# iamwinter/UMPR

Measured on AMD Instinct MI355X. Metric: training samples/sec, higher is better.
Workload: dtype f32

## Files before the change

include/umpr_hip.h:

```cpp
#ifndef UMPR_HIP_H
#define UMPR_HIP_H
#include <stddef.h>
#include <stdint.h>

#ifdef __cplusplus
extern "C" {
#endif

const char* umpr_version(void);
const char* umpr_last_error(void);
int umpr_device_info(int dev, char* name, int name_len, int* compute_units, size_t* hbm_bytes);

int umpr_gemm_f32(const float* A, long lda, int transA, const float* B, long ldb, int transB, float* C, long ldc,
                  int M, int N, int K, const float* bias, int bias_mode, int act, int accumulate, float alpha,
                  float* ws, size_t ws_bytes, void* stream);

int umpr_set_gemm_bf16(int on);

int umpr_set_conv_inference(int on);

int umpr_set_conv_pool_follows(int on);

long umpr_debug_wino_fix_count(void);

int umpr_debug_conv3x3_plan(int pass, int N, int Cin, int Cout, int H, int W, int inference, size_t* ws_bytes, size_t* v_bytes);

int umpr_debug_wino_pool_fold(const float* y, const float* g_pooled, const float* w, const float* x, float* unpooled, float* dx,
                              float* dw, float* db, int N, int Cin, int Cout, int H, int W, int f4, int fold, float* ws,
                              size_t ws_bytes, void* stream);

size_t umpr_embed_gru_bidir_ws_bytes(int N, int L, int E);
int umpr_embed_gru_bidir_fwd(const int64_t* ids, const float* emb, int E,
                             const float* w_ih_f, const float* w_hh_f, const float* b_ih_f, const float* b_hh_f,
                             const float* w_ih_r, const float* w_hh_r, const float* b_ih_r, const float* b_hh_r,
                             const int32_t* lengths, const int32_t* order, const int32_t* dst_row, int N, int L,
                             float* out, float* saved, float* ws, size_t ws_bytes, void* stream);
int umpr_embed_gru_bidir_bwd(const int64_t* ids, const float* emb, int E,
                             const float* w_hh_f, const float* w_hh_r,
                             const int32_t* lengths, const int32_t* order, const int32_t* dst_row, int N, int L,
                             const float* dout, const float* out, const float* saved,
                             float* dw_ih_f, float* dw_hh_f, float* db_ih_f, float* db_hh_f,
                             float* dw_ih_r, float* dw_hh_r, float* db_ih_r, float* db_hh_r,
                             float* ws, size_t ws_bytes, void* stream);

int umpr_embed_gru_bidir_bwd_acc(const int64_t* ids, const float* emb, int E,
                                 const float* w_hh_f, const float* w_hh_r,
                                 const int32_t* lengths, const int32_t* order, const int32_t* dst_row, int N, int L,
                                 const float* dout, const float* out, const float* saved,
                                 float* dw_ih_f, float* dw_hh_f, float* db_ih_f, float* db_hh_f,
                                 float* dw_ih_r, float* dw_hh_r, float* db_ih_r, float* db_hh_r,
                                 int accumulate, float* ws, size_t ws_bytes, void* stream);

int umpr_embed_gru_bidir_bwd_dx(const int64_t* ids, const float* emb, int E,
                                const float* w_hh_f, const float* w_hh_r,
                                const int32_t* lengths, const int32_t* order, const int32_t* dst_row, int N, int L,
                                const float* dout, const float* out, const float* saved,
                                float* dw_ih_f, float* dw_hh_f, float* db_ih_f, float* db_hh_f,
                                float* dw_ih_r, float* dw_hh_r, float* db_ih_r, float* db_hh_r,
                                int accumulate, const float* w_ih_f, const float* w_ih_r, float* dx, int dx_accumulate,
                                float* ws, size_t ws_bytes, void* stream);

int umpr_embed_grad_chunk(void);
size_t umpr_embed_grad_ws_bytes(long T, int E);
int umpr_embed_grad(const int64_t* const* ids, const float* const* dx, const long* counts, int n_src, int E, long vocab,
                    const int32_t* sorted_pos, float* d_emb, void* ws, size_t ws_bytes, void* stream);

size_t umpr_embed_grad_rows_ws_bytes(long T, int E);
int umpr_embed_grad_rows(const int64_t* const* ids, const float* const* dx, const long* counts, int n_src, int E, long vocab,
                         const int32_t* sorted_pos, int64_t* row_id, float* row_grad, void* ws, size_t ws_bytes, void* stream);
int umpr_sparse_adam_rows(float* p, float* m, float* v, long vocab, int E, const int64_t* row_id, const float* row_grad, long T,
                          double lr, double beta1, double beta2, double eps, long step, double grad_scale,
                          const float* clip_state , void* stream);

size_t umpr_coattention_fwd_ws_bytes(int B, int SL);
int umpr_coattention_fwd(const float* Gu, const float* Gi, const float* M, int B, int SL, float* T, float* soft_u,
                         float* soft_i, float* atte_u, long ld_u, float* atte_i, long ld_i, float* colmax,
                         int32_t* argcol, float* rowmax, int32_t* argrow, float* ws, size_t ws_bytes, void* stream);
int umpr_coattention_fwd_bf16(const float* Gu, const float* Gi, const float* M, int B, int SL, float* T, float* soft_u,
                              float* soft_i, float* atte_u, long ld_u, float* atte_i, long ld_i, float* colmax,
                              int32_t* argcol, float* rowmax, int32_t* argrow, float* ws, size_t ws_bytes, void* stream);
int umpr_token_mask(const int64_t* ids, const int32_t* lengths, int N, int L, long pad_id, uint8_t* valid, void* stream);
int umpr_coattention_fwd_masked(const float* Gu, const float* Gi, const float* M, int B, int SL, float* T, float* soft_u,
                                float* soft_i, float* atte_u, long ld_u, float* atte_i, long ld_i, float* colmax,
                                int32_t* argcol, float* rowmax, int32_t* argrow, const uint8_t* valid_u,
                                const uint8_t* valid_i, int bf16_scores, float* ws, size_t ws_bytes, void* stream);
size_t umpr_coattention_bwd_ws_bytes(int B, int SL);
int umpr_coattention_bwd(const float* Gu, const float* Gi, const float* M, const float* T, const float* soft_u,
                         const float* soft_i, const float* colmax, const int32_t* argcol, const float* rowmax,
                         const int32_t* argrow, const float* d_atte_u, long ld_du, const float* d_atte_i, long ld_di,
                         const float* d_soft_u, const float* d_soft_i, int B, int SL, float* dGu, float* dGi,
                         float* dM, int accumulate , float* ws, size_t ws_bytes, void* stream);

int umpr_snet_fwd(const float* X, const float* Ms, const float* Ws, const float* word_soft, int wl, int B, int S,
                  int L, float* U, float* P, float* wsum, float* self_atte, float* senti, long ld_senti, void* stream);
int umpr_snet_fwd_masked(const float* X, const float* Ms, const float* Ws, const float* word_soft, int wl, int B, int S,
                         int L, float* U, float* P, float* wsum, float* self_atte, float* senti, long ld_senti,
                         const uint8_t* valid, void* stream);
size_t umpr_snet_bwd_ws_bytes(int B, int S, int L);
int umpr_snet_bwd(const float* X, const float* Ms, const float* Ws, const float* U, const float* P, const float* wsum,
                  const float* self_atte, const float* d_senti, long ld_ds, const float* d_self_atte ,
                  int B, int S, int L, int wl, float* dX, float* dMs, float* dWs, float* d_word_soft ,
                  float* ws, size_t ws_bytes, void* stream);

int umpr_review_merge_fwd(const float* repr_u, const float* repr_i, const float* W_u, const float* W_i, int B,
                          float* out, void* stream);
size_t umpr_review_merge_bwd_ws_bytes(int B);
int umpr_review_merge_bwd(const float* repr_u, const float* repr_i, const float* W_u, const float* W_i,
                          const float* out, const float* d_out, int B, float* d_repr_u, float* d_repr_i, float* dW_u,
                          float* dW_i, float* ws, size_t ws_bytes, void* stream);

size_t umpr_cnet_head_fwd_ws_bytes(int B, int S, int L, int KS);
int umpr_cnet_head_fwd(const float* X, const float* Wc, const float* bc, const float* Wl, const float* bl, float thr,
// ... 229 lines not shown
```

umpr_amd/_lib.py:

```python
from __future__ import annotations

import ctypes
import os
import threading

import torch

_HERE = os.path.dirname(os.path.abspath(__file__))
LIB_PATH = os.path.join(_HERE, "libumpr_hip.so")

_T = {"p": ctypes.c_void_p, "i": ctypes.c_int, "l": ctypes.c_long, "z": ctypes.c_size_t, "f": ctypes.c_float,
      "d": ctypes.c_double, "u": ctypes.c_uint64}

SIGNATURES = {
    "umpr_version": ("", "s"),
    "umpr_last_error": ("", "s"),
    "umpr_device_info": ("ipipp", "i"),
    "umpr_gemm_f32": ("pliplipliiipiiifpzp", "i"),
    "umpr_embed_gru_bidir_ws_bytes": ("iii", "z"),
    "umpr_embed_gru_bidir_fwd": ("ppipppppppppppiipppzp", "i"),
    "umpr_embed_gru_bidir_bwd": ("ppipppppiippppppppppppzp", "i"),
    "umpr_embed_gru_bidir_bwd_acc": ("ppipppppiipppppppppppipzp", "i"),
    "umpr_embed_gru_bidir_bwd_dx": ("ppipppppiipppppppppppipppipzp", "i"),
    "umpr_embed_grad_chunk": ("", "i"),
# ... 28 lines not shown
    "umpr_vgg16_fwd_ws_bytes": ("i", "z"),
    "umpr_vgg16_ws_bytes": ("i", "z"),
    "umpr_vgg16_fwd": ("ppiiiuppppzp", "i"),
    "umpr_vgg16_bwd": ("ppiipppppzp", "i"),
    "umpr_vgg16_pool5_offset": ("i", "z"),
    "umpr_vgg16_set_block_callback": ("pp", "i"),
    "umpr_vgg16_wgrad_stream": ("", "p"),
    "umpr_vgg16_features_fwd": ("ppippzp", "i"),
    "umpr_vgg16_classifier_fwd": ("piiiuppppzp", "i"),
    "umpr_vgg16_classifier_bwd_ws_bytes": ("i", "z"),
    "umpr_vgg16_classifier_bwd": ("piippppppzp", "i"),
    "umpr_vgg16_features_bwd_ws_bytes": ("i", "z"),
    "umpr_vgg16_features_bwd": ("ppippppzp", "i"),
    "umpr_conv3x3_pack_bytes": ("iiiii", "z"),
    "umpr_conv3x3_fwd": ("ppppiiiiiipzp", "i"),
    "umpr_conv3x3_bwd_data": ("ppppiiiiipzp", "i"),
    "umpr_conv3x3_bwd_weight_ws_bytes": ("iiiii", "z"),
    "umpr_conv3x3_bwd_weight": ("ppppiiiiipzp", "i"),
    "umpr_maxpool2_fwd": ("ppliip", "i"),
    "umpr_maxpool2_bwd_relu": ("pppliip", "i"),
    "umpr_bf16_tensor_bytes": ("iiii", "z"),
    "umpr_bf16_from_nchw_f32": ("ppiiiip", "i"),
    "umpr_bf16_to_nchw_f32": ("ppiiiip", "i"),
    "umpr_conv3x3_bf16_ws_bytes": ("iiiii", "z"),
    "umpr_conv3x3_bf16_fwd": ("ppppiiiiiipzp", "i"),
    "umpr_conv3x3_bf16_bwd_data": ("ppppiiiiipzp", "i"),
    "umpr_conv3x3_bf16_bwd_weight": ("ppppiiiiipzp", "i"),
    "umpr_maxpool2_bf16_fwd": ("ppiiiip", "i"),
    "umpr_maxpool2_bf16_bwd_relu": ("pppiiiip", "i"),
    "umpr_vgg16_bf16_act_bytes": ("i", "z"),
    "umpr_vgg16_bf16_fwd_ws_bytes": ("i", "z"),
    "umpr_vgg16_bf16_bwd_ws_bytes": ("i", "z"),
    "umpr_vgg16_bf16_features_fwd": ("ppipppzp", "i"),
    "umpr_vgg16_bf16_features_bwd": ("ppippppzp", "i"),
    "umpr_vgg16_cls_arena_bytes": ("i", "z"),
    "umpr_vgg16_classifier_fwd_compact": ("piiiuppppzp", "i"),
    "umpr_vgg16_classifier_bwd_compact": ("piippppppzp", "i"),
    "umpr_vgg16_classifier_fwd_compact_bf16": ("piiiuppppzp", "i"),
    "umpr_vgg16_classifier_bwd_compact_bf16": ("piippppppzp", "i"),
    "umpr_concat_ids": ("pplpp", "i"),
    "umpr_review_net_arena_bytes": ("iii", "z"),
    "umpr_review_net_ws_bytes": ("iiii", "z"),
    "umpr_review_net_fwd": ("ppipppiiiiiipppzp", "i"),
    "umpr_review_net_fwd_masked": ("ppipppiiiiiipppzpp", "i"),
    "umpr_review_net_bwd": ("ppipppiiiippppzp", "i"),
    "umpr_review_net_bwd_dx": ("ppipppiiiipppppzp", "i"),
    "umpr_review_net_fwd_ex": ("ppippppiiiiiipppzpp", "i"),
    "umpr_review_net_bwd_ex": ("ppippppiiiipppppzp", "i"),
    "umpr_control_net_arena_bytes": ("iiiiiii", "z"),
    "umpr_control_net_ws_bytes": ("iiiiiiiii", "z"),
    "umpr_control_net_fwd": ("pppipppppiiiiiiiifiippppppzp", "i"),
    "umpr_control_net_bwd": ("pppipppppiiiiiiiiipppppppzp", "i"),
    "umpr_control_net_bwd_dx": ("pppipppppiiiiiiiiipppppppppzp", "i"),
    "umpr_control_net_fwd_ex": ("pppipppppppiiiiiiiifiippppppzppp", "i"),
    "umpr_control_net_bwd_ex": ("pppipppppppiiiiiiiiipppppppppzp", "i"),
    "umpr_head_fwd": ("pppppppppppppfiiipppppppp", "i"),
    "umpr_head_bwd": ("pppppppppppfiiippppppppppppppppppppp", "i"),
    "umpr_photo_resize_u8": ("pzpiiipp", "i"),
    "umpr_photo_store_slot_bytes": ("ii", "z"),
    "umpr_photo_fetch_u8": ("pzpppiiiplpp", "i"),
    "umpr_photo_fetch_augment_u8": ("pzppppiiiplplpppp", "i"),
    "umpr_feature_fetch_f32": ("pipppiiplpp", "i"),
    "umpr_review_collate": ("pplppppppplpiiiiilpppp", "i"),
    "umpr_bce_head_fwd": ("plpppiipppzp", "i"),
    "umpr_bce_head_bwd": ("plpppppiiplpppzp", "i"),
    "umpr_adam_step": ("ppppldddddldp", "i"),
    "umpr_sq_err_accumulate": ("pplpp", "i"),
    "umpr_adam_step_dev": ("pppplddd" "pp", "i"),
    "umpr_grad_norm_ws_bytes": ("", "z"),
    "umpr_grad_norm": ("ppidfppzpp", "i"),
    "umpr_adam_step_clip": ("ppppldddddld" "pp", "i"),
    "umpr_adam_step_dev_clip": ("pppplddd" "ppp", "i"),
    "umpr_adam_step_groups": ("ppppldddddld" "pp" "ppp" "ii" "p", "i"),
    "umpr_grad_accumulate": ("pppiip", "i"),
    "umpr_ema_update": ("pppidip", "i"),
    "umpr_arena_swap": ("pppip", "i"),
    "umpr_debug_poison_lds": ("pp", "i"),
    "umpr_set_gemm_bf16": ("i", "i"),
    "umpr_set_conv_inference": ("i", "i"),
    "umpr_set_conv_pool_follows": ("i", "i"),
    "umpr_debug_wino_fix_count": ("", "l"),
    "umpr_debug_conv3x3_plan": ("iiiiiiipp", "i"),
    "umpr_debug_wino_pool_fold": ("pppppppp" "iiiiiii" "pzp", "i"),
    "umpr_profile_enable": ("i", "i"),
    "umpr_profile_reset": ("", "i"),
    "umpr_profile_read": ("ippp", "i"),
}


class UmprHipError(RuntimeError):
    pass


class _Tls(threading.local):
    gemm_b16 = False


TLS = _Tls()


class _Lib:
    def __init__(self):
        if not os.path.exists(LIB_PATH):
            raise UmprHipError(
                f"{LIB_PATH} not found: build it with `python -c 'import __graft_entry__ as g; g.build()'` "
                f"(or `make -C umpr_amd/csrc`).  There is no CPU fallback.")
        self.cdll = ctypes.CDLL(LIB_PATH)
        self.fn = {}
        for name, (args, ret) in SIGNATURES.items():
            f = getattr(self.cdll, name)
            f.argtypes = [_T[c] for c in args]
            f.restype = {"i": ctypes.c_int, "z": ctypes.c_size_t, "s": ctypes.c_char_p, "p": ctypes.c_void_p,
                         "l": ctypes.c_long}[ret]
            self.fn[name] = f

    def last_error(self) -> str:
        return self.fn["umpr_last_error"]().decode()

    def call(self, name, *args):
        conv = []
        for a in args:
            if isinstance(a, torch.Tensor):
                conv.append(a.data_ptr())
            elif a is None:
                conv.append(None)
            else:
                conv.append(a)
        if TLS.gemm_b16:
            self.fn["umpr_set_gemm_bf16"](1)
            try:
                rc = self.fn[name](*conv)
            finally:
                self.fn["umpr_set_gemm_bf16"](0)
        else:
            rc = self.fn[name](*conv)
        if rc != 0:
            raise UmprHipError(f"{name} failed (rc={rc}): {self.last_error()}")

    def size(self, name, *args) -> int:
        return int(self.fn[name](*args))


_LIB = None


def lib() -> _Lib:
    global _LIB
    if _LIB is None:
        _LIB = _Lib()
    return _LIB


def stream_ptr() -> int:
    return torch.cuda.current_stream().cuda_stream


class Workspace:
    _bufs = {}

    @classmethod
    def get(cls, nbytes: int, device) -> torch.Tensor:
        key = (device.type, device.index, torch.cuda.current_stream(device).cuda_stream)
        buf = cls._bufs.get(key)
        if buf is None or buf.numel() * 4 < nbytes:
            buf = None
            cls._bufs[key] = None
# ... 5 lines not shown
```

umpr_amd/csrc/api.hip:

```cpp
#include <math.h>
#include <stdarg.h>
#include <stdlib.h>

#include <vector>

#include "../../include/umpr_hip.h"
#include "umpr_common.h"
#include "umpr_internal.h"

static thread_local char g_err[512] = "";
void umpr_set_error(const char* fmt, ...) {
  va_list ap;
  va_start(ap, fmt);
  vsnprintf(g_err, sizeof(g_err), fmt, ap);
  va_end(ap);
}

namespace {
const bool g_fc_small = umpr_env_on("UMPR_FC_SMALL");
struct ProfRec { hipEvent_t e0, e1; int family; double work; };
bool g_prof_on = false;
std::vector<ProfRec> g_prof;
std::vector<ProfRec> g_prof_pool;
double g_prof_ms[UMPR_K_COUNT] = {0}, g_prof_work[UMPR_K_COUNT] = {0};
// ... 35 lines not shown
  int cin = 3, hw = 224, ci = 0;
  for (int b = 0; b < 5; ++b) {
    for (int j = 0; j < kConvPerBlock[b]; ++j) {
      L.conv_cin[ci] = cin; L.conv_cout[ci] = kBlockCh[b]; L.conv_hw[ci] = hw; L.conv_block[ci] = b;
      L.conv_off[ci] = off;
      off += (size_t)n * kBlockCh[b] * hw * hw;
      cin = kBlockCh[b];
      ++ci;
    }
    hw /= 2;
    L.pool_off[b] = off;
    off += (size_t)n * kBlockCh[b] * hw * hw;
  }
  for (int j = 0; j < 2; ++j) { L.fc_off[j] = off; off += (size_t)n * 4096; }
  for (int j = 0; j < 2; ++j) { L.drop_off[j] = off; off += (size_t)n * 4096; }
  for (int i = 0; i < 13; ++i) {
    L.v_floats[i] = umpr_conv3x3_plan(CONV_FWD, n, L.conv_cin[i], L.conv_cout[i], L.conv_hw[i], L.conv_hw[i], false).v_floats;
    L.v_off[i] = off;
    off += L.v_floats[i];
  }
  L.total = off;
  return L;
}
}

extern "C" {

const char* umpr_version(void) { return "umpr_hip 0.1 (gfx950)"; }
const char* umpr_last_error(void) { return g_err; }

int umpr_device_info(int dev, char* name, int name_len, int* compute_units, size_t* hbm_bytes) {
  hipDeviceProp_t prop;
  if (hipGetDeviceProperties(&prop, dev) != hipSuccess) { umpr_set_error("device_info: no device %d", dev); return -1; }
  if (name && name_len > 0) { strncpy(name, prop.name, name_len - 1); name[name_len - 1] = 0; }
  if (compute_units) *compute_units = prop.multiProcessorCount;
  if (hbm_bytes) *hbm_bytes = prop.totalGlobalMem;
  return 0;
}

int umpr_gemm_f32(const float* A, long lda, int transA, const float* B, long ldb, int transB, float* C, long ldc,
                  int M, int N, int K, const float* bias, int bias_mode, int act, int accumulate, float alpha,
                  float* ws, size_t ws_bytes, void* stream) {
  UmprGemm g;
  g.A = A; g.lda = lda; g.transA = transA != 0; g.B = B; g.ldb = ldb; g.transB = transB != 0; g.C = C; g.ldc = ldc;
  g.M = M; g.N = N; g.K = K; g.bias = bias; g.bias_mode = bias_mode; g.act = act; g.accumulate = accumulate != 0;
  g.alpha = alpha; g.split_k = ws ? 0 : 1; g.ws = ws; g.ws_bytes = ws_bytes;
  return umpr_gemm(g, S(stream));
}

int umpr_set_gemm_bf16(int on) { umpr_gemm_set_b16(on != 0); return 0; }
static thread_local bool t_conv_inference = false, t_conv_pool_follows = false;
int umpr_set_conv_inference(int on) { t_conv_inference = on != 0; return 0; }
int umpr_set_conv_pool_follows(int on) { t_conv_pool_follows = on != 0; return 0; }
static ConvHints conv_hints() { ConvHints h; h.inference = t_conv_inference; h.pool_follows = t_conv_pool_follows; return h; }
long umpr_debug_wino_fix_count(void) { return umpr_wino_last_fix_count(); }
int umpr_debug_conv3x3_plan(int pass, int N, int Cin, int Cout, int H_, int W, int inference, size_t* ws_bytes, size_t* v_bytes) {
  UMPR_REQUIRE(pass >= CONV_FWD && pass <= CONV_WGRAD && N > 0 && Cin > 0 && Cout > 0 && H_ > 0 && W > 0, "conv3x3_plan: bad arguments");
  const ConvPlan p = umpr_conv3x3_plan(static_cast<ConvPass>(pass), N, Cin, Cout, H_, W, inference != 0);
  if (ws_bytes) *ws_bytes = p.ws_floats * sizeof(float);
  if (v_bytes) *v_bytes = p.v_floats * sizeof(float);
  return p.algo;
}
int umpr_debug_wino_pool_fold(const float* y, const float* g_pooled, const float* w, const float* x, float* unpooled, float* dx,
                              float* dw, float* db, int N, int Cin, int Cout, int H_, int W, int f4, int fold, float* ws,
                              size_t ws_bytes, void* stream) {
  UMPR_REQUIRE(N > 0 && Cin > 0 && Cout > 0 && H_ > 0 && W > 0 && (H_ % 2) == 0 && (W % 2) == 0 && y && g_pooled && ws,
               "debug_wino_pool_fold: bad arguments");
  UMPR_REQUIRE(fold || unpooled, "debug_wino_pool_fold: the un-folded run needs the buffer for the un-pooled gradient");
  UMPR_REQUIRE(!dx || (f4 && w), "debug_wino_pool_fold: the data gradient runs on the 4x4 tile and needs the weights");
  UMPR_REQUIRE(!dw || (x && (!f4 || ((H_ % 4) == 0 && (W % 4) == 0))), "debug_wino_pool_fold: the weight gradient on the 4x4 tile has no edge tiles");
  hipStream_t s = S(stream);
  ConvHints h;
  const float* g = g_pooled;
  if (fold) { h.pooled_dy = true; h.pool_y = y; }
  else {
    if (int rc = umpr_maxpool2_bwd_relu_impl(y, g_pooled, unpooled, (long)N * Cout, H_, W, s)) return rc;
    g = unpooled;
  }
  if (dx)
    if (int rc = umpr_wino_conv3x3(g, w, 1, nullptr, nullptr, dx, N, Cin, Cout, H_, W, 0, ws, ws_bytes / sizeof(float), true, h, s)) return rc;
  if (dw)
    if (int rc = umpr_wino_wgrad(g, x, dw, db, N, Cin, Cout, H_, W, 0, ws, ws_bytes / sizeof(float), f4 != 0, h, s)) return rc;
  return 0;
}

constexpr size_t kSlabs = 256;
namespace {
struct GruWs {
  float *gx, *wslab, *bslab;
  float* kslab; size_t kslab_bytes;
  float *stacked, *rows;
  float *wst, *bst;
  size_t bytes;
};
GruWs gru_ws(float* base, int N, int L, int pitch) {
  Carve c(base, sizeof(float));
  const size_t tiles = umpr_gru_tiles(N);
  GruWs w;
  w.gx = c.take<float>((size_t)N * L * 384); w.wslab = c.take<float>(tiles * 2 * G3 * H); w.bslab = c.take<float>(tiles * 2 * 2 * G3);
  w.wst = c.at<float>(c.off); w.bst = c.at<float>(c.off + (size_t)2 * G3 * pitch * sizeof(float));
  w.kslab_bytes = kSlabs * G3 * pitch * sizeof(float); w.kslab = c.take<float>(kSlabs * G3 * pitch);
  w.stacked = c.take<float>((size_t)2 * G3 * pitch); w.rows = c.take<float>((size_t)N * L * pitch); w.bytes = c.off;
  return w;
}
const bool g_emb_gather = umpr_env_on("UMPR_EMB_GATHER");
__global__ __launch_bounds__(256) void gather_rows_kernel(const int64_t* __restrict__ ids, const float* __restrict__ emb,
                                                          int E, int Ep, float* __restrict__ out, long rows) {
  const int lane = threadIdx.x & 63;
  for (long r = (long)blockIdx.x * 4 + (threadIdx.x >> 6); r < rows; r += (long)gridDim.x * 4) {
    const float* src = emb + ids[r] * (long)E;
    float* dst = out + r * (long)Ep;
    if ((E & 3) == 0) {
      for (int c = lane; c < E / 4; c += 64) reinterpret_cast<float4*>(dst)[c] = reinterpret_cast<const float4*>(src)[c];
    } else {
      for (int c = lane; c < Ep; c += 64) dst[c] = c < E ? src[c] : 0.f;
    }
  }
}
__global__ __launch_bounds__(256) void stack_wih_kernel(const float* __restrict__ wf, const float* __restrict__ wr,
                                                        const float* __restrict__ bf, const float* __restrict__ br, int E, int Ep,
                                                        float* __restrict__ wst, float* __restrict__ bst) {
  const int i = blockIdx.x * 256 + threadIdx.x;
  if (i < 2 * G3 * Ep) {
    const int row = i / Ep, c = i - row * Ep;
    const float* src = row < G3 ? wf + (long)row * E : wr + (long)(row - G3) * E;
    wst[i] = c < E ? src[c] : 0.f;
  }
  if (i < 2 * G3) bst[i] = i < G3 ? bf[i] : br[i - G3];
}
__global__ __launch_bounds__(256) void unstack_dwih_kernel(const float* __restrict__ stacked, int E, int Ep, float* __restrict__ df,
                                                           float* __restrict__ dr, int accumulate) {
  const int i = blockIdx.x * 256 + threadIdx.x;
  if (i >= 2 * G3 * E) return;
  const int row = i / E, c = i - row * E;
  const float v = stacked[(long)row * Ep + c];
  float* dst = row < G3 ? df + (long)row * E + c : dr + (long)(row - G3) * E + c;
  *dst = accumulate ? *dst + v : v;
}
inline int emb_pitch(int E) { return g_emb_gather ? (E + 3) & ~3 : E; }
int gather_rows(const int64_t* ids, const float* emb, int E, int Ep, float* out, long rows, hipStream_t s) {
  long blocks = (rows + 3) / 4;
  if (blocks > 16384) blocks = 16384;
  gather_rows_kernel<<<(unsigned)blocks, 256, 0, s>>>(ids, emb, E, Ep, out, rows);
  UMPR_LAUNCH_CHECK("gather_rows");
  return 0;
}
}

size_t umpr_embed_gru_bidir_ws_bytes(int N, int L, int E) { return gru_ws(nullptr, N, L, (E + 3) & ~3).bytes; }
int umpr_embed_gru_bidir_fwd(const int64_t* ids, const float* emb, int E,
                             const float* w_ih_f, const float* w_hh_f, const float* b_ih_f, const float* b_hh_f,
                             const float* w_ih_r, const float* w_hh_r, const float* b_ih_r, const float* b_hh_r,
                             const int32_t* lengths, const int32_t* order, const int32_t* dst_row, int N, int L,
                             float* out, float* saved, float* ws, size_t ws_bytes, void* stream) {
  UMPR_REQUIRE(N > 0 && L > 0 && E > 0, "embed_gru: bad shape N=%d L=%d E=%d", N, L, E);
  UMPR_REQUIRE(ws_bytes >= (size_t)N * L * 384 * sizeof(float), "embed_gru: workspace too small");
  const int Ep = emb_pitch(E);
  const GruWs W = gru_ws(ws, N, L, Ep);
  float* gx = W.gx;
  if (ws_bytes >= umpr_embed_gru_bidir_ws_bytes(N, L, E)) {
    float *wst = W.wst, *bst = W.bst;
    const hipStream_t s = S(stream);
    stack_wih_kernel<<<cdiv(2 * G3 * Ep, 256), 256, 0, s>>>(w_ih_f, w_ih_r, b_ih_f, b_ih_r, E, Ep, wst, bst);
    UMPR_LAUNCH_CHECK("stack_wih");
    UmprGemm g;
    if (g_emb_gather) {
// ... 875 lines not shown
```

umpr_amd/csrc/winograd.hip:

```cpp
#include <type_traits>

#include "umpr_common.h"
#include "umpr_internal.h"

namespace {

constexpr int WK = 32;
constexpr int WBM = 128;
constexpr int WBN = 128;

__device__ __forceinline__ void pool_window_grad(const float2 a, const float2 b, const float gy, float2& ga, float2& gb) {
  int arg = 0;
  float m = a.x;
  if (a.y > m) { m = a.y; arg = 1; }
  if (b.x > m) { m = b.x; arg = 2; }
  if (b.y > m) { m = b.y; arg = 3; }
  const float g = m > 0.f ? gy : 0.f;
  ga = make_float2(arg == 0 ? g : 0.f, arg == 1 ? g : 0.f);
  gb = make_float2(arg == 2 ? g : 0.f, arg == 3 ? g : 0.f);
}
typedef float f32x4_t __attribute__((ext_vector_type(4)));
__device__ __forceinline__ float as_loaded(float v) { asm volatile("" : "+v"(v)); return v; }
__device__ __forceinline__ float4 as_loaded(const float4 v) {
  f32x4_t q = {v.x, v.y, v.z, v.w};
// ... 1100 lines not shown
                                        float* __restrict__ o) {
  const float ea = g0 + c.a2 * g2, oa = c.a * g1 + c.a3 * g3, eb = g0 + c.b2 * g2, ob = c.b * g1 + c.b3 * g3;
  o[0] = g0; o[1] = ea + oa; o[2] = ea - oa; o[3] = eb + ob; o[4] = eb - ob; o[5] = g3;
}
template <bool EDGE, bool POOL = false>
__global__ __launch_bounds__(256) void wino4_dy_kernel(const float* __restrict__ dy, float* __restrict__ Gy, int N, int Mch, int H,
                                                       int W, long Tpad, long Tw, int Mpad, Wino4C wc, float* __restrict__ bias_part,
                                                       const float* __restrict__ pool_y = nullptr) {
  static_assert(!(EDGE && POOL), "a weight gradient on the 4x4 tile has no edge tiles");
  const int TH = (H + 3) / 4, TW = (W + 3) / 4;
  const long T = (long)N * TH * TW;
  const long total = (long)Mch * Tw;
  const long per = (long)Mpad * Tpad;
  for (long i = blockIdx.x * (long)blockDim.x + threadIdx.x; i < total; i += (long)gridDim.x * blockDim.x) {
    const long t = i % Tw;
    const int m = (int)(i / Tw);
    float* dst = Gy + (long)m * Tpad + t;
    float bsum = 0.f;
    if (t >= T) {
#pragma unroll
      for (int a = 0; a < 36; ++a) dst[(long)a * per] = 0.f;
    } else {
      const int tx = (int)(t % TW);
      const long r = t / TW;
      const int ty = (int)(r % TH), n = (int)(r / TH);
      const float* src = dy + (((long)n * Mch + m) * H + 4 * ty) * W + 4 * tx;
      float e[4][6];
      float4 pg[4];
      if (POOL) {
        const float* ysrc = pool_y + (((long)n * Mch + m) * H + 4 * ty) * W + 4 * tx;
        const float* gsrc = dy + (((long)n * Mch + m) * (H / 2) + 2 * ty) * (W / 2) + 2 * tx;
#pragma unroll
        for (int wr = 0; wr < 2; ++wr) {
          const float4 y0 = *reinterpret_cast<const float4*>(ysrc + (long)(2 * wr) * W);
          const float4 y1 = *reinterpret_cast<const float4*>(ysrc + (long)(2 * wr + 1) * W);
          const float2 gp = *reinterpret_cast<const float2*>(gsrc + (long)wr * (W / 2));
          float2 a0, b0, a1, b1;
          pool_window_grad(make_float2(y0.x, y0.y), make_float2(y1.x, y1.y), gp.x, a0, b0);
          pool_window_grad(make_float2(y0.z, y0.w), make_float2(y1.z, y1.w), gp.y, a1, b1);
          pg[2 * wr] = as_loaded(make_float4(a0.x, a0.y, a1.x, a1.y));
          pg[2 * wr + 1] = as_loaded(make_float4(b0.x, b0.y, b1.x, b1.y));
        }
      }
#pragma unroll
      for (int a = 0; a < 4; ++a) {
        if (EDGE) {
          const bool oky = 4 * ty + a < H;
          float d[4];
#pragma unroll
          for (int j = 0; j < 4; ++j) {
            const bool ok = oky && 4 * tx + j < W;
            const float v = src[ok ? (long)a * W + j : 0];
            d[j] = ok ? v : 0.f;
          }
          wino4_a(wc, d[0], d[1], d[2], d[3], e[a]);
          continue;
        }
        const float4 g = POOL ? pg[a] : *reinterpret_cast<const float4*>(src + (long)a * W);
        bsum += (g.x + g.y) + (g.z + g.w);
        wino4_a(wc, g.x, g.y, g.z, g.w, e[a]);
      }
#pragma unroll
      for (int b = 0; b < 6; ++b) {
        float o[6];
        wino4_a(wc, e[0][b], e[1][b], e[2][b], e[3][b], o);
#pragma unroll
        for (int a = 0; a < 6; ++a) dst[(long)(a * 6 + b) * per] = o[a];
      }
    }
    if (!EDGE && bias_part) {
      const float wsum = wave_sum(bsum);
      if ((threadIdx.x & 63) == 0) bias_part[i >> 6] = wsum;
    }
  }
}

__device__ __forceinline__ void wino4_gt(const Wino4C& c, const float* __restrict__ v, int stride, float* __restrict__ o) {
  const float s12 = v[stride] + v[2 * stride], d12 = v[stride] - v[2 * stride];
  const float s34 = v[3 * stride] + v[4 * stride], d34 = v[3 * stride] - v[4 * stride];
  o[0] = c.g0 * v[0] + c.ca * s12 + c.cb * s34;
  o[1] = (c.ca * c.a) * d12 + (c.cb * c.b) * d34;
  o[2] = (c.ca * c.a2) * s12 + (c.cb * c.b2) * s34 + v[5 * stride];
}
__global__ __launch_bounds__(256) void wino4_wgrad_finish_kernel(const float* __restrict__ P, int splits, int Mch, int C, int Mpad,
                                                                 int Cpad, float* __restrict__ dw, int accumulate, Wino4C wc) {
  __shared__ float red[3][36][64];
  const int cl = threadIdx.x & 63, g = threadIdx.x >> 6;
  const int chunks = (C + 63) / 64;
  const int m = blockIdx.x / chunks, c = (blockIdx.x % chunks) * 64 + cl;
  const long per = (long)Mpad * Cpad;
  const bool ok = c < C;
  float v[36];
#pragma unroll
  for (int a = 0; a < 36; ++a) {
    float acc = 0.f;
    if (ok)
      for (int sp = g; sp < splits; sp += 4) acc += P[((long)sp * 36 + a) * per + (long)m * Cpad + c];
    v[a] = acc;
  }
  if (g > 0) {
#pragma unroll
    for (int a = 0; a < 36; ++a) red[g - 1][a][cl] = v[a];
  }
  __syncthreads();
  __shared__ float outs[64 * 9];
  if (g == 0 && ok) {
#pragma unroll
    for (int a = 0; a < 36; ++a) v[a] = ((v[a] + red[0][a][cl]) + red[1][a][cl]) + red[2][a][cl];
    float gv[3][6];
#pragma unroll
    for (int b = 0; b < 6; ++b) {
      float o[3];
      wino4_gt(wc, v + b, 6, o);
      gv[0][b] = o[0]; gv[1][b] = o[1]; gv[2][b] = o[2];
    }
#pragma unroll
    for (int a = 0; a < 3; ++a) {
      float o[3];
      wino4_gt(wc, gv[a], 1, o);
      outs[cl * 9 + a * 3 + 0] = o[0]; outs[cl * 9 + a * 3 + 1] = o[1]; outs[cl * 9 + a * 3 + 2] = o[2];
    }
  }
  __syncthreads();
  const int c0 = (blockIdx.x % chunks) * 64;
  const int nout = (C - c0 < 64 ? C - c0 : 64) * 9;
  float* d = dw + ((long)m * C + c0) * 9;
  for (int i = threadIdx.x; i < nout; i += 256) d[i] = accumulate ? d[i] + outs[i] : outs[i];
}

struct WinoWgradParams {
  const float* Gy;
  const float* V;
  float* P;
  int MT, CT, Mpad, Cpad;
  long Tpad;
  int stages;
  int stages_per_split;
  int planes;
};

constexpr int WLDK = WK + 4;

template <int TN>
__global__ __launch_bounds__(256, 2) void wino_wgrad_gemm_kernel(WinoWgradParams p) {
  constexpr int LD = WLDK;
  constexpr int TM = 2;
  constexpr int BNC = 64 * TN;
  constexpr int NG = WK / 8;
  constexpr int SFLUSH = 4;
  __shared__ __attribute__((aligned(16))) float As[2][WBM * LD];
  __shared__ __attribute__((aligned(16))) float Bs[2][BNC * LD];
  const int tid = threadIdx.x, lane = tid & 63, wave = tid >> 6;
  const int wm = wave >> 1, wn = wave & 1;
  const int l31 = lane & 31, half = lane >> 5;
  long b = blockIdx.x;
  const int ct = (int)(b % p.CT); b /= p.CT;
  const int mt = (int)(b % p.MT); b /= p.MT;
  const int xi = (int)(b % p.planes);
  const int split = (int)(b / p.planes);
  const int s_begin = split * p.stages_per_split;
  const int s_end = min(p.stages, s_begin + p.stages_per_split);
  const int ns = s_end - s_begin;

  const int urow = tid >> 3, uq = tid & 7;
  const float* pa = p.Gy + ((long)xi * p.Mpad + mt * WBM + urow) * p.Tpad + (long)s_begin * WK + 4 * uq;
  const float* pb = p.V + ((long)xi * p.Cpad + ct * BNC + urow) * p.Tpad + (long)s_begin * WK + 4 * uq;
  const long rstep = 32 * p.Tpad;
  float* sa = &As[0][urow * LD + 4 * uq];
  float* sb = &Bs[0][urow * LD + 4 * uq];
  float4 ra0, ra1, ra2, ra3, rb0, rb1, rb2, rb3;
  auto lda = [&](int v, int s) { return *reinterpret_cast<const float4*>(pa + (long)s * WK + v * rstep); };
  auto ldb = [&](int v, int s) { return *reinterpret_cast<const float4*>(pb + (long)s * WK + v * rstep); };
  auto sta = [&](int v, int buf, const float4& r) { *reinterpret_cast<float4*>(sa + buf * (WBM * LD) + 32 * v * LD) = r; };
  auto stb = [&](int v, int buf, const float4& r) { *reinterpret_cast<float4*>(sb + buf * (BNC * LD) + 32 * v * LD) = r; };
  auto piece = [&](int q, int sn, int nbuf) {
    switch (q) {
      case 0: ra0 = lda(0, sn); break;
      case 1: ra1 = lda(1, sn); break;
      case 2: ra2 = lda(2, sn); break;
      case 3: ra3 = lda(3, sn); break;
      case 4: rb0 = ldb(0, sn); break;
      case 5: rb1 = ldb(1, sn); break;
      case 6: if (TN == 2) rb2 = ldb(2, sn); break;
      case 7: if (TN == 2) rb3 = ldb(3, sn); break;
      case 8: sta(0, nbuf, ra0); break;
      case 9: sta(1, nbuf, ra1); break;
      case 10: sta(2, nbuf, ra2); break;
      case 11: sta(3, nbuf, ra3); break;
      case 12: stb(0, nbuf, rb0); break;
      case 13: stb(1, nbuf, rb1); break;
      case 14: if (TN == 2) stb(2, nbuf, rb2); break;
      default: if (TN == 2) stb(3, nbuf, rb3); break;
    }
  };
  auto comp = [](const float4& v, int e) { return e == 0 ? v.x : e == 1 ? v.y : e == 2 ? v.z : v.w; };

  f32x16 acc[TM][TN], tot[TM][TN];
#pragma unroll
  for (int i = 0; i < TM; ++i)
#pragma unroll
    for (int j = 0; j < TN; ++j)
#pragma unroll
      for (int r = 0; r < 16; ++r) { acc[i][j][r] = 0.f; tot[i][j][r] = 0.f; }

#pragma unroll
  for (int q = 0; q < 16; ++q) piece(q, 0, 0);
  __syncthreads();
  for (int s0 = 0; s0 < ns; s0 += SFLUSH) {
#pragma unroll
    for (int i = 0; i < TM; ++i)
// ... 92 lines not shown
  WinoWgradGeom g;
  g.planes = f4 ? 36 : 16;
  g.T = f4 ? (long)N * ((H + 3) / 4) * ((W + 3) / 4) : (long)N * (H / 2) * (W / 2);
  g.Tpad = wino_tpad(g.T);
  g.bnc = Cin <= 64 ? 64 : WBN;
  g.MT = (Cout + WBM - 1) / WBM; g.CT = (Cin + g.bnc - 1) / g.bnc;
  g.Mpad = g.MT * WBM; g.Cpad = g.CT * g.bnc;
  g.stages = (int)(g.Tpad / WK);
  const int tiles = g.planes * g.MT * g.CT;
  const int max_splits = g.stages / 8 > 0 ? g.stages / 8 : 1;
  int splits = (kWinoWgradTargetWgs + tiles - 1) / tiles;
  if (g_wino_wgrad_rounds && (long)tiles * max_splits >= 512) {
    double best = 0.0;
    const int hi = max_splits < splits ? max_splits : splits;
    for (int sp = 1; sp <= hi; ++sp) {
      const long wgs = (long)tiles * sp;
      if (wgs < 512) continue;
      const double eff = (double)wgs / (double)((wgs + 511) / 512 * 512);
      if (eff > best) best = eff;
    }
    for (int sp = 1; sp <= hi; ++sp) {
      const long wgs = (long)tiles * sp;
      if (wgs < 512) continue;
      if ((double)wgs / (double)((wgs + 511) / 512 * 512) >= best - 0.03) { splits = sp; break; }
    }
  }
  if (splits > max_splits) splits = max_splits;
  if (splits < 1) splits = 1;
  g.stages_per_split = (g.stages + splits - 1) / splits;
  g.splits = (g.stages + g.stages_per_split - 1) / g.stages_per_split;
  g.Gy = 0; g.V = (size_t)g.planes * g.Mpad * g.Tpad; g.P = g.V + (size_t)g.planes * g.Cpad * g.Tpad;
  g.BP = g.P + (size_t)g.planes * g.splits * g.Mpad * g.Cpad; g.floats = g.BP + (size_t)g.Mpad * (g.Tpad / 64) + 64;
  return g;
}

int umpr_wino_wgrad(const float* dy, const float* x, float* dw, float* db, int N, int Cin, int Cout, int H, int W,
                    int accumulate, float* ws, size_t ws_floats, bool f4, const ConvHints& hints, hipStream_t s) {
  const WinoWgradGeom g = umpr_wino_wgrad_geom(N, Cin, Cout, H, W, f4);
  UMPR_REQUIRE(ws_floats >= g.floats, "winograd wgrad: workspace too small");
  UMPR_REQUIRE((H % 2) == 0 && (W % 2) == 0, "winograd wgrad: odd map %dx%d", H, W);
  float *Gy = ws + g.Gy, *V = ws + g.V, *P = ws + g.P, *BP = ws + g.BP;
  const bool edge = f4 && ((H % 4) != 0 || (W % 4) != 0);
  static const bool bias_fuse = umpr_env_on("UMPR_WINO_BIAS_FUSE");
  const bool fused_bias = db && f4 && !edge && bias_fuse && (g.Tpad % 64) == 0;
  const bool pooled = hints.pooled_dy;
  const float* py = hints.pool_y;
  if (pooled) UMPR_REQUIRE(py && !edge, "winograd wgrad: the pooled source needs the layer's output and whole tiles");
  if (f4 && edge)
    wino4_dy_kernel<true><<<nblk((long)Cout * g.Tpad, 16384), 256, 0, s>>>(dy, Gy, N, Cout, H, W, g.Tpad, g.Tpad, g.Mpad, wino4_consts(), nullptr);
  else if (f4 && pooled)
    wino4_dy_kernel<false, true><<<nblk((long)Cout * g.Tpad, 16384), 256, 0, s>>>(dy, Gy, N, Cout, H, W, g.Tpad, g.Tpad, g.Mpad, wino4_consts(),
                                                                                  fused_bias ? BP : nullptr, py);
  else if (f4)
    wino4_dy_kernel<false><<<nblk((long)Cout * g.Tpad, 16384), 256, 0, s>>>(dy, Gy, N, Cout, H, W, g.Tpad, g.Tpad, g.Mpad, wino4_consts(),
                                                                            fused_bias ? BP : nullptr);
  else if ((W / 2) % 2 == 0) {
    if (pooled) wino_dy_pair_kernel<true><<<nblk((long)Cout * g.Tpad / 2, 16384), 256, 0, s>>>(dy, Gy, N, Cout, H, W, g.Tpad, g.Tpad, g.Mpad, py);
    else wino_dy_pair_kernel<false><<<nblk((long)Cout * g.Tpad / 2, 16384), 256, 0, s>>>(dy, Gy, N, Cout, H, W, g.Tpad, g.Tpad, g.Mpad, nullptr);
  } else {
    if (pooled) wino_dy_kernel<true><<<nblk((long)Cout * g.Tpad, 16384), 256, 0, s>>>(dy, Gy, N, Cout, H, W, g.Tpad, g.Tpad, g.Mpad, py);
    else wino_dy_kernel<false><<<nblk((long)Cout * g.Tpad, 16384), 256, 0, s>>>(dy, Gy, N, Cout, H, W, g.Tpad, g.Tpad, g.Mpad, nullptr);
  }
  UMPR_LAUNCH_CHECK("wino_dy");
  if (hints.v_slot) {
    UMPR_REQUIRE(f4 && !edge && hints.v_slot_floats == (size_t)g.planes * g.Cpad * g.Tpad,
                 "winograd wgrad: the V slot does not match this layer (%d -> %d at %dx%d)", Cin, Cout, H, W);
    V = hints.v_slot;
  } else if (f4 && edge)
    wino4_input_kernel<true, false><<<nblk((long)g.Cpad * g.Tpad, 16384), 256, 0, s>>>(x, V, N, Cin, g.Cpad, H, W, g.Tpad, g.Tpad, wino4_consts(), nullptr, nullptr);
  else if (f4)
    wino4_input_kernel<false, false><<<nblk((long)g.Cpad * g.Tpad, 16384), 256, 0, s>>>(x, V, N, Cin, g.Cpad, H, W, g.Tpad, g.Tpad, wino4_consts(), nullptr, nullptr);
  else if ((W / 2) % 2 == 0)
    wino_input_pair_kernel<<<nblk((long)g.Cpad * g.Tpad / 2, 16384), 256, 0, s>>>(x, V, N, Cin, g.Cpad, H, W, g.Tpad, g.Tpad);
  else
    wino_input_kernel<<<nblk((long)g.Cpad * g.Tpad, 16384), 256, 0, s>>>(x, V, N, Cin, g.Cpad, H, W, g.Tpad, g.Tpad);
  UMPR_LAUNCH_CHECK("wino_input(wgrad)");
  WinoWgradParams p{Gy, V, P, g.MT, g.CT, g.Mpad, g.Cpad, g.Tpad, g.stages, g.stages_per_split, g.planes};
  {
    UmprProfScope prof(UMPR_K_WINO_WGRAD_GEMM, 2.0 * g.planes * (double)Cout * Cin * g.T, s);
    if (g.bnc == 64) wino_wgrad_gemm_kernel<1><<<(unsigned)(g.planes * g.MT * g.CT * g.splits), 256, 0, s>>>(p);
    else wino_wgrad_gemm_kernel<2><<<(unsigned)(g.planes * g.MT * g.CT * g.splits), 256, 0, s>>>(p);
  }
  UMPR_LAUNCH_CHECK("wino_wgrad_gemm");
  if (f4)
    wino4_wgrad_finish_kernel<<<(unsigned)((long)Cout * ((Cin + 63) / 64)), 256, 0, s>>>(P, g.splits, Cout, Cin, g.Mpad, g.Cpad, dw,
                                                                                     accumulate, wino4_consts());
  else if (g.splits >= 8)
    wino_wgrad_finish_wide_kernel<<<(unsigned)((long)Cout * ((Cin + 63) / 64)), 256, 0, s>>>(P, g.splits, Cout, Cin, g.Mpad, g.Cpad,
                                                                                         dw, accumulate);
  else
    wino_wgrad_finish_kernel<<<nblk((long)Cout * Cin, 4096), 256, 0, s>>>(P, g.splits, Cout, Cin, g.Mpad, g.Cpad, dw, accumulate);
  UMPR_LAUNCH_CHECK("wino_wgrad_finish");
  if (fused_bias) {
    wino_bias_sum_waves_kernel<<<(unsigned)((Cout + 3) / 4), 256, 0, s>>>(BP, db, Cout, g.Tpad / 64, accumulate);
    UMPR_LAUNCH_CHECK("wino_bias_sum_waves");
  } else if (db) {
    UMPR_REQUIRE((size_t)N * Cout <= (size_t)g.splits * g.planes * g.Mpad * g.Cpad && ((long)H * W) % 4 == 0,
                 "winograd wgrad: bias-gradient scratch");
    if (pooled) wino_bias_part_wave_kernel<true><<<(unsigned)(((long)N * Cout + 3) / 4), 256, 0, s>>>(dy, P, (long)H * W, (long)N * Cout, py, W);
    else wino_bias_part_wave_kernel<false><<<(unsigned)(((long)N * Cout + 3) / 4), 256, 0, s>>>(dy, P, (long)H * W, (long)N * Cout, nullptr, W);
    UMPR_LAUNCH_CHECK("wino_bias_part");
    wino_bias_sum_kernel<<<(Cout + 255) / 256, 256, 0, s>>>(P, db, N, Cout, accumulate);
    UMPR_LAUNCH_CHECK("wino_bias_sum");
  }
  return 0;
}
```

Before: 2187.

## Vectorize Winograd 4x4 wgrad finish reduction and specialize small split counts

Rewrites the F(4,3) weight-gradient finish kernel so each thread loads float4 slices of the per-split partial planes and reduces them in registers, with a 384-thread variant for many splits. Small split counts get templated 192-thread variants that handle two output rows per block. The aim is fewer scalar global loads and better bandwidth use in the partial-sum reduction, at the cost of more shared memory and added code paths. A debug entry point for the wgrad path is also added.

```diff
diff --git a/include/umpr_hip.h b/include/umpr_hip.h
--- a/include/umpr_hip.h
+++ b/include/umpr_hip.h
@@ -28,6 +28,9 @@
 int umpr_debug_wino_pool_fold(const float* y, const float* g_pooled, const float* w, const float* x, float* unpooled, float* dx,
                               float* dw, float* db, int N, int Cin, int Cout, int H, int W, int f4, int fold, float* ws,
                               size_t ws_bytes, void* stream);
+
+int umpr_debug_wino_wgrad(const float* dy, const float* x, float* dw, float* db, int N, int Cin, int Cout, int H, int W, int f4,
+                          int accumulate, float* ws, size_t ws_bytes, void* stream);
 
 size_t umpr_embed_gru_bidir_ws_bytes(int N, int L, int E);
 int umpr_embed_gru_bidir_fwd(const int64_t* ids, const float* emb, int E,
diff --git a/umpr_amd/_lib.py b/umpr_amd/_lib.py
--- a/umpr_amd/_lib.py
+++ b/umpr_amd/_lib.py
@@ -134,6 +134,7 @@
     "umpr_debug_wino_fix_count": ("", "l"),
     "umpr_debug_conv3x3_plan": ("iiiiiiipp", "i"),
     "umpr_debug_wino_pool_fold": ("pppppppp" "iiiiiii" "pzp", "i"),
+    "umpr_debug_wino_wgrad": ("pppp" "iiiiiii" "pzp", "i"),
     "umpr_profile_enable": ("i", "i"),
     "umpr_profile_reset": ("", "i"),
     "umpr_profile_read": ("ippp", "i"),
diff --git a/umpr_amd/csrc/api.hip b/umpr_amd/csrc/api.hip
--- a/umpr_amd/csrc/api.hip
+++ b/umpr_amd/csrc/api.hip
@@ -141,6 +141,16 @@
   if (dw)
     if (int rc = umpr_wino_wgrad(g, x, dw, db, N, Cin, Cout, H_, W, 0, ws, ws_bytes / sizeof(float), f4 != 0, h, s)) return rc;
   return 0;
+}
+int umpr_debug_wino_wgrad(const float* dy, const float* x, float* dw, float* db, int N, int Cin, int Cout, int H_, int W, int f4,
+                          int accumulate, float* ws, size_t ws_bytes, void* stream) {
+  UMPR_REQUIRE(N > 0 && Cin > 0 && Cout > 0 && H_ > 0 && W > 0 && (H_ % 2) == 0 && (W % 2) == 0 && dy && x && dw && ws,
+               "debug_wino_wgrad: bad arguments");
+  UMPR_REQUIRE(!f4 || ((H_ % 4) == 0 && (W % 4) == 0), "debug_wino_wgrad: the weight gradient on the 4x4 tile has no edge tiles");
+  if (int rc = umpr_wino_wgrad(dy, x, dw, db, N, Cin, Cout, H_, W, accumulate, ws, ws_bytes / sizeof(float), f4 != 0, ConvHints(),
+                               S(stream)))
+    return rc;
+  return umpr_wino_wgrad_geom(N, Cin, Cout, H_, W, f4 != 0).splits;
 }
 
 constexpr size_t kSlabs = 256;
diff --git a/umpr_amd/csrc/winograd.hip b/umpr_amd/csrc/winograd.hip
--- a/umpr_amd/csrc/winograd.hip
+++ b/umpr_amd/csrc/winograd.hip
@@ -1206,50 +1206,99 @@
   o[1] = (c.ca * c.a) * d12 + (c.cb * c.b) * d34;
   o[2] = (c.ca * c.a2) * s12 + (c.cb * c.b2) * s34 + v[5 * stride];
 }
-__global__ __launch_bounds__(256) void wino4_wgrad_finish_kernel(const float* __restrict__ P, int splits, int Mch, int C, int Mpad,
-                                                                 int Cpad, float* __restrict__ dw, int accumulate, Wino4C wc) {
-  __shared__ float red[3][36][64];
-  const int cl = threadIdx.x & 63, g = threadIdx.x >> 6;
+__device__ __forceinline__ float4 add4(const float4 a, const float4 b) { return make_float4(a.x + b.x, a.y + b.y, a.z + b.z, a.w + b.w); }
+template <int NS>
+__global__ __launch_bounds__(NS == 0 ? 384 : 192) void wino4_wgrad_finish_kernel(const float* __restrict__ P, int splits, int Mch, int C,
+                                                                               int Mpad, int Cpad, float* __restrict__ dw,
+                                                                               int accumulate, Wino4C wc) {
+  constexpr int GT = NS == 0 ? 4 : 1, ROWS = GT == 4 ? 1 : 2;
+  __shared__ float4 part[ROWS][4][36][16];
+  __shared__ float outs[ROWS][64 * 9];
+  const int l = threadIdx.x & 15, b = (threadIdx.x >> 4) % 6, z = threadIdx.x / 96;
   const int chunks = (C + 63) / 64;
-  const int m = blockIdx.x / chunks, c = (blockIdx.x % chunks) * 64 + cl;
+  const int c0 = (blockIdx.x % chunks) * 64, m0 = (blockIdx.x / chunks) * ROWS;
   const long per = (long)Mpad * Cpad;
-  const bool ok = c < C;
-  float v[36];
-#pragma unroll
-  for (int a = 0; a < 36; ++a) {
-    float acc = 0.f;
-    if (ok)
-      for (int sp = g; sp < splits; sp += 4) acc += P[((long)sp * 36 + a) * per + (long)m * Cpad + c];
-    v[a] = acc;
-  }
-  if (g > 0) {
-#pragma unroll
-    for (int a = 0; a < 36; ++a) red[g - 1][a][cl] = v[a];
+  const float4 zero = make_float4(0.f, 0.f, 0.f, 0.f);
+  {
+    const int row = GT == 4 ? 0 : z;
+    const bool live = m0 + row < Mch && c0 + 4 * l < C;
+    const float* src = P + (long)b * per + (long)(m0 + row) * Cpad + c0 + 4 * l;
+    if (GT == 4) {
+      float4 acc[6];
+#pragma unroll
+      for (int a = 0; a < 6; ++a) acc[a] = zero;
+      if (live)
+        for (int sp = z; sp < splits; sp += 8) {
+          const bool two = sp + 4 < splits;
+          float4 x0[6], x1[6];
+#pragma unroll
+          for (int a = 0; a < 6; ++a) x0[a] = *reinterpret_cast<const float4*>(src + ((long)sp * 36 + 6 * a) * per);
+          if (two) {
+#pragma unroll
+            for (int a = 0; a < 6; ++a) x1[a] = *reinterpret_cast<const float4*>(src + ((long)(sp + 4) * 36 + 6 * a) * per);
+          }
+#pragma unroll
+          for (int a = 0; a < 6; ++a) acc[a] = add4(acc[a], x0[a]);
+          if (two) {
+#pragma unroll
+            for (int a = 0; a < 6; ++a) acc[a] = add4(acc[a], x1[a]);
+          }
+        }
+#pragma unroll
+      for (int a = 0; a < 6; ++a) part[0][z][6 * a + b][l] = acc[a];
+    } else {
+      float4 x[3][6];
+#pragma unroll
+      for (int q = 0; q < 3; ++q)
+#pragma unroll
+        for (int a = 0; a < 6; ++a) x[q][a] = zero;
+      if (live) {
+#pragma unroll
+        for (int q = 0; q < NS; ++q)
+#pragma unroll
+          for (int a = 0; a < 6; ++a) x[q][a] = *reinterpret_cast<const float4*>(src + ((long)q * 36 + 6 * a) * per);
+      }
+#pragma unroll
+      for (int a = 0; a < 6; ++a) {
+#pragma unroll
+        for (int q = 0; q < 3; ++q) part[row][q][6 * a + b][l] = add4(zero, x[q][a]);
+        part[row][3][6 * a + b][l] = zero;
+      }
+    }
   }
   __syncthreads();
-  __shared__ float outs[64 * 9];
-  if (g == 0 && ok) {
-#pragma unroll
-    for (int a = 0; a < 36; ++a) v[a] = ((v[a] + red[0][a][cl]) + red[1][a][cl]) + red[2][a][cl];
-    float gv[3][6];
-#pragma unroll
-    for (int b = 0; b < 6; ++b) {
-      float o[3];
-      wino4_gt(wc, v + b, 6, o);
-      gv[0][b] = o[0]; gv[1][b] = o[1]; gv[2][b] = o[2];
-    }
-#pragma unroll
-    for (int a = 0; a < 3; ++a) {
-      float o[3];
-      wino4_gt(wc, gv[a], 1, o);
-      outs[cl * 9 + a * 3 + 0] = o[0]; outs[cl * 9 + a * 3 + 1] = o[1]; outs[cl * 9 + a * 3 + 2] = o[2];
+  {
+    const int cl = threadIdx.x & 63, row = threadIdx.x >> 6;
+    const int m = m0 + row, c = c0 + cl;
+    const bool ok = c < C;
+    if (row < ROWS && m < Mch && ok) {
+      const float* red = reinterpret_cast<const float*>(&part[row][0][0][0]);
+      float v[36];
+#pragma unroll
+      for (int a = 0; a < 36; ++a) v[a] = red[a * 64 + cl];
+#pragma unroll
+      for (int a = 0; a < 36; ++a) v[a] = ((v[a] + red[(36 + a) * 64 + cl]) + red[(72 + a) * 64 + cl]) + red[(108 + a) * 64 + cl];
+      float gv[3][6];
+#pragma unroll
+      for (int b = 0; b < 6; ++b) {
+        float o[3];
+        wino4_gt(wc, v + b, 6, o);
+        gv[0][b] = o[0]; gv[1][b] = o[1]; gv[2][b] = o[2];
+      }
+#pragma unroll
+      for (int a = 0; a < 3; ++a) {
+        float o[3];
+        wino4_gt(wc, gv[a], 1, o);
+        outs[row][cl * 9 + a * 3 + 0] = o[0]; outs[row][cl * 9 + a * 3 + 1] = o[1]; outs[row][cl * 9 + a * 3 + 2] = o[2];
+      }
     }
   }
   __syncthreads();
-  const int c0 = (blockIdx.x % chunks) * 64;
   const int nout = (C - c0 < 64 ? C - c0 : 64) * 9;
-  float* d = dw + ((long)m * C + c0) * 9;
-  for (int i = threadIdx.x; i < nout; i += 256) d[i] = accumulate ? d[i] + outs[i] : outs[i];
+  for (int r = 0; r < ROWS && m0 + r < Mch; ++r) {
+    float* d = dw + ((long)(m0 + r) * C + c0) * 9;
+    for (int i = threadIdx.x; i < nout; i += blockDim.x) d[i] = accumulate ? d[i] + outs[r][i] : outs[r][i];
+  }
 }
 
 struct WinoWgradParams {
@@ -1508,9 +1557,18 @@
     else wino_wgrad_gemm_kernel<2><<<(unsigned)(g.planes * g.MT * g.CT * g.splits), 256, 0, s>>>(p);
   }
   UMPR_LAUNCH_CHECK("wino_wgrad_gemm");
-  if (f4)
-    wino4_wgrad_finish_kernel<<<(unsigned)((long)Cout * ((Cin + 63) / 64)), 256, 0, s>>>(P, g.splits, Cout, Cin, g.Mpad, g.Cpad, dw,
-                                                                                     accumulate, wino4_consts());
+  if (f4) {
+    const long chunks = (Cin + 63) / 64;
+    const unsigned pairs = (unsigned)((Cout + 1) / 2 * chunks);
+    if (g.splits >= 4)
+      wino4_wgrad_finish_kernel<0><<<(unsigned)(Cout * chunks), 384, 0, s>>>(P, g.splits, Cout, Cin, g.Mpad, g.Cpad, dw, accumulate, wino4_consts());
+    else if (g.splits == 3)
+      wino4_wgrad_finish_kernel<3><<<pairs, 192, 0, s>>>(P, g.splits, Cout, Cin, g.Mpad, g.Cpad, dw, accumulate, wino4_consts());
+    else if (g.splits == 2)
+      wino4_wgrad_finish_kernel<2><<<pairs, 192, 0, s>>>(P, g.splits, Cout, Cin, g.Mpad, g.Cpad, dw, accumulate, wino4_consts());
+    else
+      wino4_wgrad_finish_kernel<1><<<pairs, 192, 0, s>>>(P, g.splits, Cout, Cin, g.Mpad, g.Cpad, dw, accumulate, wino4_consts());
+  }
   else if (g.splits >= 8)
     wino_wgrad_finish_wide_kernel<<<(unsigned)((long)Cout * ((Cin + 63) / 64)), 256, 0, s>>>(P, g.splits, Cout, Cin, g.Mpad, g.Cpad,
                                                                                          dw, accumulate);
```

Result: no change. 2198, median of 6 (+0.5%).
